# Improbable-AI/walk-these-ways

Measured on AMD Instinct MI355X. Metric: env-steps/sec (sim+PPO), higher is better.
Workload: dtype f32

## Files before the change

### include/go1ppo.h

```cpp
#ifndef GO1PPO_H
#define GO1PPO_H
#include <stdint.h>

#ifdef __cplusplus
extern "C" {
#endif

#define GO1PPO_ABI_VERSION 3
#define GO1PPO_MAX_ACTIONS 32

int go1ppo_elu_fwd(void* y, int64_t rows, int cols, int ld, const void* lat, int lat_ld, int npv, const void* wz,
                   int wz_ld, int lat_cols, void* stream);

int go1ppo_elu_bwd(const void* d, int ld_d, const void* h, int ld_h, int64_t rows, int cols, float* bias_grad, void* out,
                   int ld_out, void* stream);

typedef struct {
  const void* mean;
  const void* value;
  const float* std;
  int32_t head_ld, num_actions;
  int64_t rows;
  const int64_t* idx;
  const float* actions;
// ... 112 lines not shown
                    int64_t count1, float gscale, const float* partial, float max_norm, const float* step, const float* lr,
                    float beta1, float beta2, float eps, void* body, int64_t n_body, float* tail, int64_t n_tail, int zero_grad,
                    float* zero_slot, const Go1PpoAdamExtras* extras, void* stream);

int go1ppo_sum_partials(const void* partials, int count, int64_t stride, int64_t rows, int cols, float* out, int zero_rows,
                        int zero_c0, int zero_c1, void* stream);


typedef struct Go1PpoGemmArgs {
  const void* A; const void* B; void* C; const float* bias; const void* H;
  int32_t M, N, K, lda, ldb, ldc, ldh, epilogue, elu_c0, elu_c1;
  int32_t elu_skip_c0, elu_skip_c1;
  int32_t bias_bf16, _pad;
} Go1PpoGemmArgs;
int go1ppo_gemm_nt(const Go1PpoGemmArgs* args, void* stream);
int go1ppo_gemm_nt_pair(const Go1PpoGemmArgs* a, const Go1PpoGemmArgs* b, void* stream);

int go1ppo_wgrad_tn_plan(Go1PpoWgradProblem* problems, int count);
int go1ppo_wgrad_tn_batched(const Go1PpoWgradProblem* device_problems, int count, int total_workgroups, void* stream);

#define GO1PPO_MLP2_MAX_NETS 3
typedef struct {
  void* x;
  const void* W2; const void* b2;
  const void* W3; const void* b3;
  void* z2;
  void* out;
  int64_t rows;
  int32_t ld_x, ld_z2, ld_out, elu_input;
} Go1PpoMlp2Fwd;
int go1ppo_mlp2_fwd(const Go1PpoMlp2Fwd* nets, int count, void* stream);

typedef struct {
  const void* d_out;
  const void* z2; const void* h;
  const void* W2; const void* W3;
  void* d_z2;
  void* d_x;
  int64_t rows;
  int32_t ld_dout, ld_z2, ld_h, ld_dz2, ld_dx, _pad;
} Go1PpoMlp2Bwd;
int go1ppo_mlp2_bwd(const Go1PpoMlp2Bwd* nets, int count, void* stream);

typedef struct {
  void* x;
  const void* W2; const void* b2;
  const void* W3; const void* b3;
  void* z2;
  void* out;
  void* d_out;
  void* d_z2;
  void* d_x;
  int64_t rows;
  int32_t ld_x, ld_z2, ld_out, ld_dout, ld_dz2, ld_dx, elu_input, _pad;
} Go1PpoMlp2Tail;

#define GO1PPO_TAIL_MAX_ACTIONS 12
int go1ppo_mlp2_tail_ppo(const Go1PpoMlp2Tail* nets, const Go1PpoLossArgs* loss, void* stream);

typedef struct {
  const float* target;
  const int64_t* idx;
  int64_t num_train;
  int32_t npv, selective;
  float* d_pred_bias;
  float* train_loss;
// ... 11 lines not shown
```

### walk-these-ways_amd/csrc/go1ppo_mlp.h

```cpp
#pragma once

#define MLP2_K1 256
#define MLP2_N2 128
#define MLP2_N3 64
#define MLP2_BM 64
#define MLP2_WAVES 16
#define MLP2_THREADS (64 * MLP2_WAVES)
#define MLP2_IMG (128 * 128)

struct Mlp2FwdArgs { Go1PpoMlp2Fwd net[GO1PPO_MLP2_MAX_NETS]; };
struct Mlp2BwdArgs { Go1PpoMlp2Bwd net[GO1PPO_MLP2_MAX_NETS]; };

__device__ __forceinline__ int swz_row(int row) { return row & 15; }
__device__ __forceinline__ int swz_red(int row) { return 2 * ((row & 3) | (((row >> 3) & 1) << 2)); }

template <bool RED>
__device__ __forceinline__ void dma_weights(const bf16_t* W, int rows, int cols, bf16_t* img, int wave, int lane) {
  const int windows = cols >> 7, count = (rows >> 2) * windows;
  for (int idx = wave; idx < count; idx += MLP2_WAVES) {
    const int win = idx % windows, blk = idx / windows;
    const int row = blk * 4 + (lane >> 4);
    const int chunk = (lane & 15) ^ (RED ? swz_red(row) : swz_row(row));
    glds16(W + (int64_t)row * cols + win * 128 + chunk * 8, img + win * MLP2_IMG + blk * 4 * 128);
  }
}

__device__ __forceinline__ uint2 pack_bf4(const float (&v)[4]) {
  f32x2 lo = {v[0], v[1]}, hi = {v[2], v[3]};
  uint2 o;
  o.x = __builtin_bit_cast(uint32_t, __builtin_convertvector(lo, bf16x2_t));
  o.y = __builtin_bit_cast(uint32_t, __builtin_convertvector(hi, bf16x2_t));
  return o;
}
__device__ __forceinline__ void unpack_bf4(uint2 r, float (&v)[4]) {
  v[0] = __uint_as_float(r.x << 16); v[1] = __uint_as_float(r.x & 0xffff0000u);
  v[2] = __uint_as_float(r.y << 16); v[3] = __uint_as_float(r.y & 0xffff0000u);
}
__device__ __forceinline__ bf16x8_t lds_b128(const bf16_t* img, int byte_off) {
  return *reinterpret_cast<const bf16x8_t*>(reinterpret_cast<const char*>(img) + byte_off);
}
__device__ __forceinline__ bf16x8_t lds_tr_operand(const bf16_t* img, int byte_off) {
  typedef __attribute__((address_space(3))) s16x4_t lds_s16x4_t;
  const char* p = reinterpret_cast<const char*>(img) + byte_off;
  s16x4_t lo = __builtin_amdgcn_ds_read_tr16_b64_v4i16((lds_s16x4_t*)(p));
  s16x4_t hi = __builtin_amdgcn_ds_read_tr16_b64_v4i16((lds_s16x4_t*)(p + 4 * 256));
  s16x8_t v = __builtin_shufflevector(lo, hi, 0, 1, 2, 3, 4, 5, 6, 7);
  return __builtin_bit_cast(bf16x8_t, v);
}

__global__ __launch_bounds__(MLP2_THREADS, 1) void mlp2_fwd_kernel(Mlp2FwdArgs A) {
  __shared__ __attribute__((aligned(1024))) bf16_t W2i[2 * MLP2_IMG];
  __shared__ __attribute__((aligned(1024))) bf16_t W3i[64 * 128];
  __shared__ __attribute__((aligned(1024))) bf16_t Ai[2 * 64 * 128];
  __shared__ __attribute__((aligned(1024))) bf16_t Z2i[64 * 128];
  const Go1PpoMlp2Fwd& N = A.net[blockIdx.y];
  const int tiles = (int)((N.rows + MLP2_BM - 1) / MLP2_BM);
  if ((int)blockIdx.x >= tiles) return;
  const int t = threadIdx.x, wave = t >> 6, lane = t & 63, r = lane & 15, g = lane >> 4;
  dma_weights<false>((const bf16_t*)N.W2, MLP2_N2, MLP2_K1, W2i, wave, lane);
  dma_weights<false>((const bf16_t*)N.W3, MLP2_N3, MLP2_N2, W3i, wave, lane);
  bf16_t* x = (bf16_t*)N.x;
  bf16_t* z2 = (bf16_t*)N.z2;
  bf16_t* out = (bf16_t*)N.out;
  const int tx = g ^ r;
  int foff[4];
#pragma unroll
  for (int a = 0; a < 4; a++) foff[a] = r * 256 + (((4 * a) ^ tx) << 4);
  const int nf2 = wave >> 1, mp = (wave & 1) * 2, nf3 = wave & 3, m3 = wave >> 2;
  float bias2[4], bias3[4];
  unpack_bf4(*reinterpret_cast<const uint2*>((const bf16_t*)N.b2 + nf2 * 16 + 4 * g), bias2);
  unpack_bf4(*reinterpret_cast<const uint2*>((const bf16_t*)N.b3 + nf3 * 16 + 4 * g), bias3);

  Bf8 v[2];
  auto fetch = [&](int tile) {
#pragma unroll
    for (int j = 0; j < 2; j++) {
      const int p = t + MLP2_THREADS * j, row = p >> 5, ch = p & 31;
      int64_t grow = (int64_t)tile * MLP2_BM + row;
      grow = grow < N.rows ? grow : N.rows - 1;
      v[j] = *reinterpret_cast<const Bf8*>(x + grow * N.ld_x + ch * 8);
    }
  };
  fetch(blockIdx.x);
  bool first = true;
  for (int tile = blockIdx.x; tile < tiles; tile += gridDim.x) {
    const int64_t row0 = (int64_t)tile * MLP2_BM;
#pragma unroll
    for (int j = 0; j < 2; j++) {
      const int p = t + MLP2_THREADS * j, row = p >> 5, ch = p & 31;
      if (N.elu_input) {
        float f[8];
#pragma unroll
        for (int e = 0; e < 8; e++) f[e] = elu1(bf2f(v[j].v[e]));
        v[j] = pack_bf8(f);
        if (row0 + row < N.rows) *reinterpret_cast<Bf8*>(x + (row0 + row) * N.ld_x + ch * 8) = v[j];
      }
      *reinterpret_cast<Bf8*>(reinterpret_cast<char*>(Ai + (ch >> 4) * 64 * 128) + row * 256 + (((ch & 15) ^ swz_row(row)) << 4)) = v[j];
    }
    if (first) asm volatile("s_waitcnt vmcnt(0)" ::: "memory");
    first = false;
    __syncthreads();
    if (tile + (int)gridDim.x < tiles) fetch(tile + gridDim.x);
    {
      f32x4 acc[2] = {f32x4{0.f, 0.f, 0.f, 0.f}, f32x4{0.f, 0.f, 0.f, 0.f}};
#pragma unroll
      for (int ks = 0; ks < MLP2_K1 / 32; ks++) {
        const int win = ks >> 2, off = foff[ks & 3];
        const bf16x8_t w = lds_b128(W2i + win * MLP2_IMG + nf2 * 16 * 128, off);
#pragma unroll
        for (int m = 0; m < 2; m++)
          acc[m] = __builtin_amdgcn_mfma_f32_16x16x32_bf16(w, lds_b128(Ai + win * 64 * 128 + (mp + m) * 16 * 128, off), acc[m], 0, 0, 0);
      }
      const int n0 = nf2 * 16 + 4 * g;
#pragma unroll
      for (int m = 0; m < 2; m++) {
        const int row = (mp + m) * 16 + r;
        float o4[4];
#pragma unroll
        for (int e = 0; e < 4; e++) o4[e] = elu1(acc[m][e] + bias2[e]);
        const uint2 o = pack_bf4(o4);
        if (row0 + row < N.rows) *reinterpret_cast<uint2*>(z2 + (row0 + row) * N.ld_z2 + n0) = o;
        *reinterpret_cast<uint2*>(reinterpret_cast<char*>(Z2i) + row * 256 + (((n0 >> 3) ^ swz_row(row)) << 4) + ((n0 >> 2) & 1) * 8) = o;
      }
    }
    __syncthreads();
    {
      f32x4 acc = f32x4{0.f, 0.f, 0.f, 0.f};
#pragma unroll
      for (int ks = 0; ks < MLP2_N2 / 32; ks++)
        acc = __builtin_amdgcn_mfma_f32_16x16x32_bf16(lds_b128(W3i + nf3 * 16 * 128, foff[ks]), lds_b128(Z2i + m3 * 16 * 128, foff[ks]), acc, 0, 0, 0);
      const int n0 = nf3 * 16 + 4 * g, row = m3 * 16 + r;
      float o4[4];
#pragma unroll
      for (int e = 0; e < 4; e++) o4[e] = acc[e] + bias3[e];
      if (row0 + row < N.rows) *reinterpret_cast<uint2*>(out + (row0 + row) * N.ld_out + n0) = pack_bf4(o4);
    }
  }
}

__global__ __launch_bounds__(MLP2_THREADS, 1) void mlp2_bwd_kernel(Mlp2BwdArgs A) {
  __shared__ __attribute__((aligned(1024))) bf16_t W3t[64 * 128];
  __shared__ __attribute__((aligned(1024))) bf16_t W2t[2 * MLP2_IMG];
  __shared__ __attribute__((aligned(1024))) bf16_t D3i[64 * 128];
  __shared__ __attribute__((aligned(1024))) bf16_t D2i[64 * 128];
  __shared__ __attribute__((aligned(1024))) bf16_t Hi[2 * 64 * 128];
  const Go1PpoMlp2Bwd& N = A.net[blockIdx.y];
  const int tiles = (int)((N.rows + MLP2_BM - 1) / MLP2_BM);
  if ((int)blockIdx.x >= tiles) return;
  const int t = threadIdx.x, wave = t >> 6, lane = t & 63, r = lane & 15, g = lane >> 4;
  dma_weights<true>((const bf16_t*)N.W3, MLP2_N3, MLP2_N2, W3t, wave, lane);
  dma_weights<true>((const bf16_t*)N.W2, MLP2_N2, MLP2_K1, W2t, wave, lane);
  const bf16_t* d = (const bf16_t*)N.d_out;
  const bf16_t* z2 = (const bf16_t*)N.z2;
  const bf16_t* hin = (const bf16_t*)N.h;
  bf16_t* dz2 = (bf16_t*)N.d_z2;
  bf16_t* dx = (bf16_t*)N.d_x;
  const int tx = g ^ r;
  int foff[4];
#pragma unroll
  for (int a = 0; a < 4; a++) foff[a] = r * 256 + (((4 * a) ^ tx) << 4);
  const int troff = (g * 8 + (r >> 2)) * 256 + ((r & 3) >> 1) * 16 + (r & 1) * 8;
  const int swb = 32 * ((r >> 2) | ((g & 1) << 2));
  const int kf2 = wave >> 1, mp = (wave & 1) * 2;
  const int w3off = troff + (((kf2 * 16) * 2) ^ swb);
  const bf16_t* w2img = W2t + (wave >> 3) * MLP2_IMG;
  const int w2off = troff + ((((wave & 7) * 16) * 2) ^ swb);
  const int hch = t & 31;
#define MLP2_HROW(j) ((t + (j) * MLP2_THREADS) >> 5)
  const int zrow = t >> 4, zch = t & 15, drow = (t >> 3) & 63, dch = t & 7;
#define MLP2_HSLOT(j) ((hch >> 4) * (64 * 128 * 2) + MLP2_HROW(j) * 256 + (((hch & 15) ^ swz_row(MLP2_HROW(j))) << 4))
// ... 493 lines not shown
    });
  }
}

template <int AMAX>
__global__ __launch_bounds__(MLP2_THREADS, 1) void mlp2_tail_ppo_kernel(Mlp2TailPpoArgs A) {
  mlp2_tail_body<0, AMAX>(A.net[blockIdx.y], A.loss, Go1PpoMseArgs{});
}
__global__ __launch_bounds__(MLP2_THREADS, 1) void mlp2_tail_mse_kernel(Mlp2TailMseArgs A) {
  mlp2_tail_body<1, 4>(A.net, Go1PpoLossArgs{}, A.mse);
}

static inline bool aligned8(const void* p) { return (reinterpret_cast<uintptr_t>(p) & 7) == 0; }

extern "C" int go1ppo_mlp2_fwd(const Go1PpoMlp2Fwd* nets, int count, void* stream) {
  if (!nets || count <= 0 || count > GO1PPO_MLP2_MAX_NETS) return -1;
  Mlp2FwdArgs A;
  int64_t max_rows = 0;
  for (int i = 0; i < count; i++) {
    const Go1PpoMlp2Fwd& N = nets[i];
    if (!N.x || !N.W2 || !N.b2 || !N.W3 || !N.b3 || !N.z2 || !N.out || N.rows <= 0) return -1;
    if ((N.ld_x & 7) || (N.ld_z2 & 3) || (N.ld_out & 3) || N.ld_x < MLP2_K1 || N.ld_z2 < MLP2_N2 || N.ld_out < MLP2_N3 || !aligned16(N.x) ||
        !aligned16(N.W2) || !aligned16(N.W3) || !aligned8(N.b2) || !aligned8(N.b3) || !aligned8(N.z2) || !aligned8(N.out))
      return -2;
    A.net[i] = N;
    if (N.rows > max_rows) max_rows = N.rows;
  }
  int64_t wgs = (max_rows + MLP2_BM - 1) / MLP2_BM;
  if (wgs > 256 / count) wgs = 256 / count;
  mlp2_fwd_kernel<<<dim3((unsigned)wgs, count), dim3(MLP2_THREADS), 0, (hipStream_t)stream>>>(A);
  return hipGetLastError() == hipSuccess ? 0 : -9;
}

extern "C" int go1ppo_mlp2_bwd(const Go1PpoMlp2Bwd* nets, int count, void* stream) {
  if (!nets || count <= 0 || count > GO1PPO_MLP2_MAX_NETS) return -1;
  Mlp2BwdArgs A;
  int64_t max_rows = 0;
  for (int i = 0; i < count; i++) {
    const Go1PpoMlp2Bwd& N = nets[i];
    if (!N.d_out || !N.z2 || !N.h || !N.W2 || !N.W3 || !N.d_z2 || !N.d_x || N.rows <= 0) return -1;
    if ((N.ld_dout & 7) || (N.ld_z2 & 7) || (N.ld_h & 7) || (N.ld_dz2 & 7) || (N.ld_dx & 7) || N.ld_dout < MLP2_N3 || N.ld_z2 < MLP2_N2 ||
        N.ld_h < MLP2_K1 || N.ld_dz2 < MLP2_N2 || N.ld_dx < MLP2_K1 || !aligned16(N.d_out) || !aligned16(N.W2) || !aligned16(N.W3) ||
        !aligned16(N.z2) || !aligned16(N.h) || !aligned16(N.d_z2) || !aligned16(N.d_x))
      return -2;
    A.net[i] = N;
    if (N.rows > max_rows) max_rows = N.rows;
  }
  int64_t wgs = (max_rows + MLP2_BM - 1) / MLP2_BM;
  if (wgs > 256 / count) wgs = 256 / count;
  mlp2_bwd_kernel<<<dim3((unsigned)wgs, count), dim3(MLP2_THREADS), 0, (hipStream_t)stream>>>(A);
  return hipGetLastError() == hipSuccess ? 0 : -9;
}

static int mlp2_tail_check(const Go1PpoMlp2Tail& N) {
  if (!N.x || !N.W2 || !N.b2 || !N.W3 || !N.b3 || !N.z2 || !N.out || !N.d_out || !N.d_z2 || !N.d_x || N.rows <= 0) return -1;
  if ((N.rows + MLP2_BM - 1) / MLP2_BM > DET_TAIL_MAX_TILES) return -1;
  return 0;
}
static int mlp2_tail_check_shape(const Go1PpoMlp2Tail& N) {
  if ((N.ld_x & 7) || (N.ld_z2 & 7) || (N.ld_dz2 & 7) || (N.ld_dx & 7) || N.ld_x < MLP2_K1 || N.ld_z2 < MLP2_N2 || N.ld_dz2 < MLP2_N2 ||
      N.ld_dx < MLP2_K1 || N.ld_out != MLP2_N3 || N.ld_dout != MLP2_N3 || !aligned16(N.x) || !aligned16(N.W2) || !aligned16(N.W3) ||
      !aligned8(N.b2) || !aligned8(N.b3) || !aligned16(N.z2) || !aligned16(N.out) || !aligned16(N.d_out) || !aligned16(N.d_z2) ||
      !aligned16(N.d_x) || N.d_z2 == N.z2 || N.d_x == N.x)
    return -2;
  return 0;
}
// ... 43 lines not shown
```

### walk-these-ways_amd/go1_gym_learn/ppo_cse/fused.py

```python
import ctypes
import os

import torch

HEAD = 64
_HERE = os.path.dirname(os.path.abspath(__file__))
_LIB_PATH = os.path.normpath(os.path.join(_HERE, "..", "..", "csrc", "libgo1ppo.so"))
_lib = None


class Go1PpoLibraryMissing(RuntimeError):
    pass


class LossArgs(ctypes.Structure):
    _fields_ = [("mean", ctypes.c_void_p), ("value", ctypes.c_void_p), ("std", ctypes.c_void_p),
                ("head_ld", ctypes.c_int32), ("num_actions", ctypes.c_int32), ("rows", ctypes.c_int64),
                ("idx", ctypes.c_void_p), ("actions", ctypes.c_void_p), ("old_mu", ctypes.c_void_p),
                ("old_sigma", ctypes.c_void_p), ("old_logp", ctypes.c_void_p), ("advantages", ctypes.c_void_p),
                ("returns", ctypes.c_void_p), ("old_values", ctypes.c_void_p),
                ("clip_param", ctypes.c_float), ("value_loss_coef", ctypes.c_float), ("entropy_coef", ctypes.c_float),
                ("use_clipped_value_loss", ctypes.c_int32),
                ("d_mean", ctypes.c_void_p), ("d_value", ctypes.c_void_p), ("d_std", ctypes.c_void_p),
                ("d_mean_bias", ctypes.c_void_p), ("d_value_bias", ctypes.c_void_p), ("kl", ctypes.c_void_p),
# ... 5 lines not shown
                ("rows", ctypes.c_int64), ("ld_dz", ctypes.c_int32), ("ld_h", ctypes.c_int32), ("n", ctypes.c_int32),
                ("k", ctypes.c_int32), ("ldw", ctypes.c_int32), ("chunk_rows", ctypes.c_int32), ("wg_offset", ctypes.c_int32),
                ("zero_n", ctypes.c_int32), ("zero_k0", ctypes.c_int32), ("zero_k1", ctypes.c_int32),
                ("partials", ctypes.c_void_p), ("partial_stride", ctypes.c_int64)]


class GradPiece(ctypes.Structure):
    _fields_ = [("begin", ctypes.c_int64), ("count", ctypes.c_int64), ("src", ctypes.c_void_p), ("stride", ctypes.c_int64),
                ("kind", ctypes.c_int32), ("slabs", ctypes.c_int32), ("cols", ctypes.c_int32), ("zero_rows", ctypes.c_int32),
                ("zero_c0", ctypes.c_int32), ("zero_c1", ctypes.c_int32)]


class TailLayer(ctypes.Structure):
    _fields_ = [("W", ctypes.c_void_p), ("bias", ctypes.c_void_p), ("out", ctypes.c_void_p), ("n_out", ctypes.c_int32),
                ("k_in", ctypes.c_int32), ("ld_out", ctypes.c_int32), ("elu", ctypes.c_int32)]


class TailNet(ctypes.Structure):
    _fields_ = [("in_", ctypes.c_void_p), ("rows", ctypes.c_int64), ("ld_in", ctypes.c_int32), ("num_layers", ctypes.c_int32),
                ("elu_in", ctypes.c_int32), ("npv", ctypes.c_int32), ("latent", ctypes.c_void_p), ("wz", ctypes.c_void_p),
                ("lat_ld", ctypes.c_int32), ("wz_ld", ctypes.c_int32),
                ("layer", TailLayer * 4)]


class TailArgs(ctypes.Structure):
    _fields_ = [("num_nets", ctypes.c_int32), ("_pad", ctypes.c_int32), ("net", TailNet * 3)]


class Mlp2Fwd(ctypes.Structure):
    _fields_ = [(n, ctypes.c_void_p) for n in ("x", "W2", "b2", "W3", "b3", "z2", "out")] + [("rows", ctypes.c_int64)] + \
               [(n, ctypes.c_int32) for n in ("ld_x", "ld_z2", "ld_out", "elu_input")]


class Mlp2Bwd(ctypes.Structure):
    _fields_ = [(n, ctypes.c_void_p) for n in ("d_out", "z2", "h", "W2", "W3", "d_z2", "d_x")] + [("rows", ctypes.c_int64)] + \
               [(n, ctypes.c_int32) for n in ("ld_dout", "ld_z2", "ld_h", "ld_dz2", "ld_dx", "_pad")]


class Mlp2Tail(ctypes.Structure):
    _fields_ = [(n, ctypes.c_void_p) for n in ("x", "W2", "b2", "W3", "b3", "z2", "out", "d_out", "d_z2", "d_x")] + [("rows", ctypes.c_int64)] + \
               [(n, ctypes.c_int32) for n in ("ld_x", "ld_z2", "ld_out", "ld_dout", "ld_dz2", "ld_dx", "elu_input", "_pad")]


class MseArgs(ctypes.Structure):
    _fields_ = [("target", ctypes.c_void_p), ("idx", ctypes.c_void_p), ("num_train", ctypes.c_int64), ("npv", ctypes.c_int32),
                ("selective", ctypes.c_int32), ("d_pred_bias", ctypes.c_void_p), ("train_loss", ctypes.c_void_p), ("test_loss", ctypes.c_void_p)]


MLP2_DIMS = (256, 128, 64)
TAIL_MAX_ACTIONS = 12


class GemmArgs(ctypes.Structure):
    _fields_ = [("A", ctypes.c_void_p), ("B", ctypes.c_void_p), ("C", ctypes.c_void_p), ("bias", ctypes.c_void_p),
                ("H", ctypes.c_void_p)] + [(n, ctypes.c_int32) for n in
                                           ("M", "N", "K", "lda", "ldb", "ldc", "ldh", "epilogue", "elu_c0", "elu_c1", "elu_skip_c0", "elu_skip_c1", "bias_bf16", "_pad")]


class _AdamTranspose(ctypes.Structure):
    _fields_ = [("start", ctypes.c_int64), ("rows", ctypes.c_int32), ("cols", ctypes.c_int32), ("dst", ctypes.c_void_p)]


class AdamExtras(ctypes.Structure):
    _fields_ = [("num_transposes", ctypes.c_int32), ("_pad", ctypes.c_int32), ("transpose", _AdamTranspose * 2)]


EXPORTED_SYMBOLS = ["go1ppo_mlp2_fwd", "go1ppo_mlp2_bwd", "go1ppo_mlp2_tail_ppo", "go1ppo_mlp2_tail_mse", "go1ppo_gemm_nt", "go1ppo_gemm_nt_pair", "go1ppo_sum_partials", "go1ppo_wgrad_tn_plan", "go1ppo_wgrad_tn_batched", "go1ppo_tail_fwd", "go1ppo_elu_fwd", "go1ppo_elu_bwd", "go1ppo_loss", "go1ppo_mse", "go1ppo_wgrad", "go1ppo_wgrad_plan",
                    "go1ppo_wgrad_batched", "go1ppo_act",
                    "go1ppo_store_step", "go1ppo_ring_snapshot", "go1ppo_ring_step", "go1ppo_ring_gather", "go1ppo_gae", "go1ppo_normalize", "go1ppo_opt_partials", "go1ppo_opt_prestep",
                    "go1ppo_opt_prestep_pieces", "go1ppo_grad_reduce", "go1ppo_opt_adam", "go1ppo_version"]


def load_library(path=None):
    global _lib
    if _lib is not None and path is None:
        return _lib
    p = path or _LIB_PATH
    if not os.path.exists(p):
        raise Go1PpoLibraryMissing(f"{p} not found: run `python -c 'import __graft_entry__ as g; g.build()'` "
                                   "(hipcc --offload-arch=gfx950); the fused PPO update has no CPU fallback")
    L = ctypes.CDLL(p)
    vp, i32, i64 = ctypes.c_void_p, ctypes.c_int, ctypes.c_int64
    L.go1ppo_elu_fwd.argtypes = [vp, i64, i32, i32, vp, i32, i32, vp, i32, i32, vp]
    L.go1ppo_elu_bwd.argtypes = [vp, i32, vp, i32, i64, i32, vp, vp, i32, vp]
    L.go1ppo_loss.argtypes = [ctypes.POINTER(LossArgs), vp]
    L.go1ppo_mse.argtypes = [vp, i32, vp, i32, vp, i64, i64, i32, vp, vp, vp, vp, vp]
    L.go1ppo_wgrad.argtypes = [vp, i32, vp, i32, i64, i32, i32, vp, i32, vp, vp]
    L.go1ppo_wgrad_plan.argtypes = [ctypes.POINTER(WgradProblem), i32]
    L.go1ppo_tail_fwd.argtypes = [ctypes.POINTER(TailArgs), vp]
    L.go1ppo_gemm_nt.argtypes = [ctypes.POINTER(GemmArgs), vp]
    L.go1ppo_gemm_nt_pair.argtypes = [ctypes.POINTER(GemmArgs), ctypes.POINTER(GemmArgs), vp]
    L.go1ppo_sum_partials.argtypes = [vp, i32, i64, i64, i32, vp, i32, i32, i32, vp]
    L.go1ppo_mlp2_fwd.argtypes = [ctypes.POINTER(Mlp2Fwd), i32, vp]
    L.go1ppo_mlp2_bwd.argtypes = [ctypes.POINTER(Mlp2Bwd), i32, vp]
    L.go1ppo_mlp2_tail_ppo.argtypes = [ctypes.POINTER(Mlp2Tail), ctypes.POINTER(LossArgs), vp]
    L.go1ppo_mlp2_tail_mse.argtypes = [ctypes.POINTER(Mlp2Tail), ctypes.POINTER(MseArgs), vp]
    L.go1ppo_wgrad_batched.argtypes = [vp, i32, i32, vp]
    L.go1ppo_wgrad_tn_plan.argtypes = [ctypes.POINTER(WgradProblem), i32]
    L.go1ppo_wgrad_tn_batched.argtypes = [vp, i32, i32, vp]
    f32 = ctypes.c_float
    L.go1ppo_act.argtypes = [vp, vp, i32, vp, i32, i64, vp, vp, vp, vp, vp, vp, vp]
    L.go1ppo_store_step.argtypes = [vp, vp, vp, vp, vp, f32, i64, vp, vp, vp, vp]
    L.go1ppo_ring_snapshot.argtypes = [vp, i64, i64, i32, i32, vp, vp]
    L.go1ppo_ring_step.argtypes = [vp, vp, vp, vp, i64, i32, i32, i32, i32, vp, vp, vp, vp]
    L.go1ppo_ring_gather.argtypes = [vp, vp, vp, i64, i64, i32, i32, i32, i32, vp, vp]
    L.go1ppo_gae.argtypes = [vp, vp, vp, vp, i32, i64, f32, f32, vp, vp, vp, vp]
    L.go1ppo_normalize.argtypes = [vp, i64, vp, vp]
    L.go1ppo_opt_partials.argtypes = []
    L.go1ppo_opt_prestep.argtypes = [vp, i64, f32, vp, vp, vp, vp, f32, f32, f32, f32, vp]
    L.go1ppo_opt_prestep_pieces.argtypes = [vp, i64, vp, i32, f32, vp, vp, vp, vp, f32, f32, f32, f32, vp]
    L.go1ppo_grad_reduce.argtypes = [vp, vp, i32, vp]
    L.go1ppo_opt_adam.argtypes = [vp, vp, vp, vp, i64, i64, i64, i64, f32, vp, f32, vp, vp, f32, f32, f32, vp, i64, vp, i64, i32, vp,
                                  ctypes.POINTER(AdamExtras), vp]
    for name in EXPORTED_SYMBOLS[:-1]:
        getattr(L, name).restype = ctypes.c_int
    L.go1ppo_version.restype = ctypes.c_char_p
    if path is None:
        _lib = L
    return L


def _stream():
    return torch.cuda.current_stream().cuda_stream


def _chk(rc, what):
# ... 11 lines not shown


def gemm_args(a, b, c, bias=None, elu=None, elu_bwd_of=None, elu_skip=None):
    g = GemmArgs()
    g.A, g.B, g.C, g.bias, g.H = a.data_ptr(), b.data_ptr(), c.data_ptr(), _ptr(bias), _ptr(elu_bwd_of)
    g.M, g.N, g.K, g.lda, g.ldb, g.ldc = a.shape[0], b.shape[0], a.shape[1], _ld(a), _ld(b), _ld(c)
    assert b.shape[1] == g.K and tuple(c.shape) == (g.M, g.N) and (elu is None or elu_bwd_of is None)
    assert a.dtype == b.dtype == c.dtype == torch.bfloat16 and (bias is None or bias.dtype in (torch.float32, torch.bfloat16))
    g.bias_bf16 = int(bias is not None and bias.dtype == torch.bfloat16)
    if elu_bwd_of is not None:
        assert elu_bwd_of.shape == c.shape and elu_bwd_of.dtype == torch.bfloat16
        g.epilogue, g.ldh = 2, _ld(elu_bwd_of)
    elif elu is not None:
        g.epilogue = 1
        g.elu_c0, g.elu_c1 = (0, g.N) if elu is True else elu
        if elu_skip is not None:
            g.elu_skip_c0, g.elu_skip_c1 = elu_skip
    return g


def gemm_nt(lib, a, b, c, bias=None, elu=None, elu_bwd_of=None):
    g = gemm_args(a, b, c, bias, elu, elu_bwd_of)
    _chk(lib.go1ppo_gemm_nt(ctypes.byref(g), _stream()), "go1ppo_gemm_nt")
    return c


def gemm_nt_pair(lib, first, second):
    ga, gb = gemm_args(**first), gemm_args(**second)
    _chk(lib.go1ppo_gemm_nt_pair(ctypes.byref(ga), ctypes.byref(gb), _stream()), "go1ppo_gemm_nt_pair")


class FusedNet:

    def __init__(self, policy, body, grad, M, lib, with_grad, two_streams=True, fused_tails=None):
        assert body.dtype == torch.bfloat16 and body.is_cuda
        self.pol, self.M, self.lib = policy, M, lib
        dev = body.device
        self.P = {name: policy._block(body, name) for name, _ in policy.blocks}
        self.G = {name: policy._block(grad, name) for name, _ in policy.blocks} if grad is not None else None
        self.nd, self.na, self.nc = policy.first
        self.n1 = self.nd + self.na + self.nc
        self.depth = {n: len(l) for n, l in policy.nets.items()}
        bf = dict(device=dev, dtype=torch.bfloat16)
        self.Y1 = torch.zeros(M, self.n1, **bf)
        self.Y1d = torch.zeros(M, self.nd, **bf)
        self.Z = {n: {li: torch.zeros(M, self.P[f"{n}.{li}.W"].shape[0], **bf) for li in range(1, d)}
                  for n, d in self.depth.items()}
        assert policy.npv <= HEAD and self.P["Wz"].shape == (self.na, HEAD)
        self._recording, self._batched, self._plans = None, False, {}
        self._grad = grad
        self.defer_grad_sum = False
        self._rec_pieces, self._slab_ws, self._last_pieces = None, {}, {}
        self._wgrad_tn = M % 64 == 0
        self._tails = self._tails_ad = None
        if fused_tails is None:
            fused_tails = M <= int(os.environ.get("GO1_FUSED_TAILS_MAX_ROWS", "2048"))
        self._elu_on_load = not with_grad
        if fused_tails and self._fused_tails_ok():
            nd, na = self.nd, self.na
            eol = self._elu_on_load
            self._tails = (self._tail_args([("adaptation", self.Y1[:, :nd])], with_grad, elu_in=eol),
                           self._tail_args([("actor", self.Y1[:, nd:nd + na]), ("critic", self.Y1[:, nd + na:])], with_grad, elu_in=eol,
                                           latent_for="actor" if eol else None))
            self._tails_ad = self._tail_args([("adaptation", self.Y1d)], with_grad)
        self._mlp2 = (self._tails is None and os.environ.get("GO1_MLP2", "1") == "1" and self.nd == MLP2_DIMS[0] and
                      all(self.depth[n] >= 3 and tuple(self.P[f"{n}.{self.depth[n] - 2}.W"].shape) == (MLP2_DIMS[1], MLP2_DIMS[0])
                          and tuple(self.P[f"{n}.{self.depth[n] - 1}.W"].shape) == (MLP2_DIMS[2], MLP2_DIMS[1]) for n in self.depth)
                      and self.depth["adaptation"] == 3 and self.depth["actor"] == 4 and self.depth["critic"] == 4)
        self._mlp2_cache = {}
        self._tail_in_loss = False
        na1, nc1 = int(self.P["actor.1.W"].shape[0]), int(self.P["critic.1.W"].shape[0])
        nt_ok = all(v % 64 == 0 for v in (na1, nc1, self.na, self.n1 - self.nd - self.na)) and \
            all(self.P[k].data_ptr() % 16 == 0 for k in ("actor.1.b", "critic.1.b", "actor.1.W", "critic.1.W"))
        pair_ok = nt_ok and na1 == nc1 and self.na == self.n1 - self.nd - self.na
        self._l1_nt = nt_ok
        self._pair = pair_ok
        self._side = torch.cuda.Stream(device=dev) if two_streams else None
        if with_grad:
            self.X = torch.zeros(M, policy.Kp, **bf)
            self.dH1 = {"adaptation": torch.zeros(M, self.nd, **bf), "actor": torch.zeros(M, self.na, **bf),
                        "critic": torch.zeros(M, self.nc, **bf)}
            self.dY1 = torch.zeros(M, self.n1, **bf)
            self.dZ = {n: {li: torch.zeros_like(z) for li, z in zs.items()} for n, zs in self.Z.items()}
            w1_split = next((b for b in (M // 6144, 4, 2) if b >= 2 and M % b == 0 and (M // b) % 64 == 0), 1)
            self._w1_tmp = torch.zeros(w1_split, self.n1, policy.Kp, **bf)
            self._dgrad_nt = self._mlp2 and nt_ok
            self._WT = {n: torch.zeros(self.P[f"{n}.1.W"].shape[1], self.P[f"{n}.1.W"].shape[0], **bf) for n in ("actor", "critic")} \
                if self._dgrad_nt else None
            self._wt_by_optimizer = False
            self.priv_mask = (self.nd + self.na, policy.K + 1, policy.K + 1 + policy.npv)

    def _elu(self, y, lat=None, lat_cols=0):
        wz = self.P["Wz"] if lat is not None else None
        _chk(self.lib.go1ppo_elu_fwd(y.data_ptr(), y.shape[0], y.shape[1], _ld(y), _ptr(lat), _ld(lat) if lat is not None else 0,
                                     self.pol.npv if lat is not None else 0, _ptr(wz), HEAD, lat_cols, _stream()), "go1ppo_elu_fwd")

    def _elu_bwd(self, d, h, bias_grad, out=None):
        out = d if out is None else out
        _chk(self.lib.go1ppo_elu_bwd(d.data_ptr(), _ld(d), _ptr(h), _ld(h) if h is not None else 0, d.shape[0], d.shape[1],
                                     _ptr(bias_grad), out.data_ptr(), _ld(out), _stream()), "go1ppo_elu_bwd")

    def _wgrad(self, dz, h, gW, gb=None, zero=None):
# ... 39 lines not shown
        for li in range(1, d):
            z = self.Z[net][li]
            torch.addmm(P[f"{net}.{li}.b"], h, P[f"{net}.{li}.W"].t(), out=z)
            if li < d - 1:
                self._elu(z)
            h = z
        return h

    def forward(self, x):
        nd, na = self.nd, self.na
        if self._mlp2:
            return self._forward_mlp2(x)
        torch.mm(x, self.P["W1"].t(), out=self.Y1)
        if self._tails is not None:
            ta, tac = self._tails
            if not self._elu_on_load:
                self._elu(self.Y1[:, :nd])
            _chk(self.lib.go1ppo_tail_fwd(ctypes.byref(ta), _stream()), "go1ppo_tail_fwd")
            latent = self.Z["adaptation"][self.depth["adaptation"] - 1]
            if not self._elu_on_load:
                self._elu(self.Y1[:, nd:], latent, na)
            _chk(self.lib.go1ppo_tail_fwd(ctypes.byref(tac), _stream()), "go1ppo_tail_fwd")
            return self.Z["actor"][self.depth["actor"] - 1], self.Z["critic"][self.depth["critic"] - 1], latent
        self._elu(self.Y1[:, :nd])
        latent = self._tail("adaptation", self.Y1[:, :nd])
        self._elu(self.Y1[:, nd:], latent, na)
        with self._branch():
            value = self._tail("critic", self.Y1[:, nd + na:])
        mean = self._tail("actor", self.Y1[:, nd:nd + na])
        self._join()
        return mean, value, latent

    def _mlp2_fwd(self, key, items, elu_input=1):
        key = ("fwd", key, elu_input)
        if key not in self._mlp2_cache:
            arr = (Mlp2Fwd * len(items))()
            for a, (net, x) in zip(arr, items):
                d = self.depth[net]
                W2, W3, z2, out = self.P[f"{net}.{d - 2}.W"], self.P[f"{net}.{d - 1}.W"], self.Z[net][d - 2], self.Z[net][d - 1]
                a.x, a.W2, a.b2, a.W3, a.b3 = x.data_ptr(), W2.data_ptr(), self.P[f"{net}.{d - 2}.b"].data_ptr(), W3.data_ptr(), self.P[f"{net}.{d - 1}.b"].data_ptr()
                a.z2, a.out, a.rows, a.ld_x, a.ld_z2, a.ld_out, a.elu_input = z2.data_ptr(), out.data_ptr(), x.shape[0], _ld(x), _ld(z2), _ld(out), int(elu_input)
            self._mlp2_cache[key] = (arr, len(items))
        arr, n = self._mlp2_cache[key]
        _chk(self.lib.go1ppo_mlp2_fwd(arr, n, _stream()), "go1ppo_mlp2_fwd")

    def _mlp2_bwd(self, key, items):
        key = ("bwd", key)
        if key not in self._mlp2_cache:
            arr = (Mlp2Bwd * len(items))()
            for a, (net, h, d_x) in zip(arr, items):
                d = self.depth[net]
                d_out, z2, d_z2 = self.dZ[net][d - 1], self.Z[net][d - 2], self.dZ[net][d - 2]
                a.d_out, a.z2, a.h, a.W2, a.W3 = d_out.data_ptr(), z2.data_ptr(), h.data_ptr(), self.P[f"{net}.{d - 2}.W"].data_ptr(), self.P[f"{net}.{d - 1}.W"].data_ptr()
                a.d_z2, a.d_x, a.rows = d_z2.data_ptr(), d_x.data_ptr(), h.shape[0]
                a.ld_dout, a.ld_z2, a.ld_h, a.ld_dz2, a.ld_dx = _ld(d_out), _ld(z2), _ld(h), _ld(d_z2), _ld(d_x)
            self._mlp2_cache[key] = (arr, len(items))
        arr, n = self._mlp2_cache[key]
        _chk(self.lib.go1ppo_mlp2_bwd(arr, n, _stream()), "go1ppo_mlp2_bwd")

    def _mlp2_tail(self, key, items):
        key = ("tail", key)
        if key not in self._mlp2_cache:
            arr = (Mlp2Tail * len(items))()
            for a, (net, x, d_x) in zip(arr, items):
                d = self.depth[net]
                W2, W3, z2, out = self.P[f"{net}.{d - 2}.W"], self.P[f"{net}.{d - 1}.W"], self.Z[net][d - 2], self.Z[net][d - 1]
                d_out, d_z2 = self.dZ[net][d - 1], self.dZ[net][d - 2]
                a.x, a.W2, a.b2, a.W3, a.b3 = x.data_ptr(), W2.data_ptr(), self.P[f"{net}.{d - 2}.b"].data_ptr(), W3.data_ptr(), self.P[f"{net}.{d - 1}.b"].data_ptr()
                a.z2, a.out, a.d_out, a.d_z2, a.d_x, a.rows = z2.data_ptr(), out.data_ptr(), d_out.data_ptr(), d_z2.data_ptr(), d_x.data_ptr(), x.shape[0]
                a.ld_x, a.ld_z2, a.ld_out, a.ld_dout, a.ld_dz2, a.ld_dx, a.elu_input = _ld(x), _ld(z2), _ld(out), _ld(d_out), _ld(d_z2), _ld(d_x), 1
            self._mlp2_cache[key] = arr
        return self._mlp2_cache[key]

    def _tail_ok(self, arr):
        for a in arr:
            if a.ld_out != HEAD or a.ld_dout != HEAD or a.ld_x % 8 or a.ld_z2 % 8 or a.ld_dz2 % 8 or a.ld_dx % 8 or a.d_x == a.x or a.d_z2 == a.z2:
                return False
            if any(p % 16 for p in (a.x, a.W2, a.W3, a.z2, a.out, a.d_out, a.d_z2, a.d_x)) or a.b2 % 8 or a.b3 % 8:
                return False
        return True

    def tail_ppo_fused(self, num_actions):
        if not (self._mlp2 and self.G is not None and 0 < num_actions <= TAIL_MAX_ACTIONS):
            return False
        Z, dZ = self.Z, self.dZ
        return self._tail_ok(self._mlp2_tail("ac", [("actor", Z["actor"][1], dZ["actor"][1]), ("critic", Z["critic"][1], dZ["critic"][1])]))

    def tail_adaptation_fused(self):
        if not (self._mlp2 and self.G is not None):
            return False
        return self._tail_ok(self._mlp2_tail("adaptation_only", [("adaptation", self.Y1d, self.dH1["adaptation"])]))

    def _forward_mlp2(self, x):
        P, Z, nd, na = self.P, self.Z, self.nd, self.na
        torch.mm(x, P["W1"].t(), out=self.Y1)
        self._mlp2_fwd("adaptation", [("adaptation", self.Y1[:, :nd])])
        latent = Z["adaptation"][2]
        self._elu(self.Y1[:, nd:], latent, na)
        if self._l1_nt and self._pair:
            gemm_nt_pair(self.lib, dict(a=self.Y1[:, nd:nd + na], b=P["actor.1.W"], c=Z["actor"][1], bias=P["actor.1.b"]),
                         dict(a=self.Y1[:, nd + na:], b=P["critic.1.W"], c=Z["critic"][1], bias=P["critic.1.b"]))
        elif self._l1_nt:
            with self._branch():
                gemm_nt(self.lib, self.Y1[:, nd + na:], P["critic.1.W"], Z["critic"][1], P["critic.1.b"])
            gemm_nt(self.lib, self.Y1[:, nd:nd + na], P["actor.1.W"], Z["actor"][1], P["actor.1.b"])
        else:
            with self._branch():
                torch.addmm(P["critic.1.b"], self.Y1[:, nd + na:], P["critic.1.W"].t(), out=Z["critic"][1])
            torch.addmm(P["actor.1.b"], self.Y1[:, nd:nd + na], P["actor.1.W"].t(), out=Z["actor"][1])
        self._join()
        if not self._tail_in_loss:
            self._mlp2_fwd("ac", [("actor", Z["actor"][1]), ("critic", Z["critic"][1])])
        return Z["actor"][3], Z["critic"][3], latent

    def _backward_mlp2(self, x):
        nd, na = self.nd, self.na
        P, G, Z, dZ, Y1, dY1, dH1 = self.P, self.G, self.Z, self.dZ, self.Y1, self.dY1, self.dH1
        cols = {"adaptation": slice(0, nd), "actor": slice(nd, nd + na), "critic": slice(nd + na, self.n1)}
        if not self._tail_in_loss:
            self._mlp2_bwd("ac", [("actor", Z["actor"][1], dZ["actor"][1]), ("critic", Z["critic"][1], dZ["critic"][1])])
        for net in ("actor", "critic"):
            self._wgrad(dZ[net][3], Z[net][2], G[f"{net}.3.W"], None)
            self._wgrad(dZ[net][2], Z[net][1], G[f"{net}.2.W"], G[f"{net}.2.b"])
            self._wgrad(dZ[net][1], Y1[:, cols[net]], G[f"{net}.1.W"], G[f"{net}.1.b"])
        if self._dgrad_nt and self._pair and self._wt_by_optimizer:
            gemm_nt_pair(self.lib, dict(a=dZ["actor"][1], b=self._WT["actor"], c=dY1[:, cols["actor"]], elu_bwd_of=Y1[:, cols["actor"]]),
                         dict(a=dZ["critic"][1], b=self._WT["critic"], c=dY1[:, cols["critic"]], elu_bwd_of=Y1[:, cols["critic"]]))
        elif self._dgrad_nt:
            with self._branch():
                if not self._wt_by_optimizer:
                    self._WT["critic"].copy_(P["critic.1.W"].t())
# ... 353 lines not shown
```

Measured before the change: 5.332 million.

## Fold latent-injection ELU pass into adaptation MLP2 forward kernel

Adds a templated variant of the adaptation MLP2 forward kernel that, besides computing the adaptation latent, also applies the latent-weight injection and ELU to the rest of the first-layer activation block. Each workgroup finishes its own tile's latent-dependent columns from LDS and streams the latent-free columns of another tile while it waits on memory. This removes a separate ELU kernel launch and a round trip of the latent through global memory. It is enabled by default only for large batches, and falls back to the old path if alignment checks fail. The cost is more LDS use, software prefetch of the next tile is moved later, and the kernel code is considerably more complex.

```diff
diff --git a/include/go1ppo.h b/include/go1ppo.h
--- a/include/go1ppo.h
+++ b/include/go1ppo.h
@@ -168,6 +168,13 @@
 int go1ppo_mlp2_fwd(const Go1PpoMlp2Fwd* nets, int count, void* stream);
 
 typedef struct {
+  void* y;
+  const void* wz;
+  int32_t cols, ld, lat_cols, npv, wz_ld, _pad;
+} Go1PpoEluBlock;
+int go1ppo_mlp2_fwd_elu(const Go1PpoMlp2Fwd* net, const Go1PpoEluBlock* blk, void* stream);
+
+typedef struct {
   const void* d_out;
   const void* z2; const void* h;
   const void* W2; const void* W3;
diff --git a/walk-these-ways_amd/csrc/go1ppo_mlp.h b/walk-these-ways_amd/csrc/go1ppo_mlp.h
--- a/walk-these-ways_amd/csrc/go1ppo_mlp.h
+++ b/walk-these-ways_amd/csrc/go1ppo_mlp.h
@@ -48,12 +48,20 @@
   return __builtin_bit_cast(bf16x8_t, v);
 }
 
-__global__ __launch_bounds__(MLP2_THREADS, 1) void mlp2_fwd_kernel(Mlp2FwdArgs A) {
+#define ELU_U 4
+#define ELU_WZ_LDS_COLS 2048
+struct Mlp2FwdEluArgs { Go1PpoMlp2Fwd net; Go1PpoEluBlock blk; };
+struct EluWalk { int row, ch; };
+struct EluCols { int c0, cpr, q, rm; };
+
+template <bool FOLD>
+__device__ __forceinline__ void mlp2_fwd_body(const Go1PpoMlp2Fwd& N, const Go1PpoEluBlock& E) {
   __shared__ __attribute__((aligned(1024))) bf16_t W2i[2 * MLP2_IMG];
   __shared__ __attribute__((aligned(1024))) bf16_t W3i[64 * 128];
   __shared__ __attribute__((aligned(1024))) bf16_t Ai[2 * 64 * 128];
   __shared__ __attribute__((aligned(1024))) bf16_t Z2i[64 * 128];
-  const Go1PpoMlp2Fwd& N = A.net[blockIdx.y];
+  __shared__ __attribute__((aligned(16))) bf16_t Hd[FOLD ? 64 * 64 : 8];
+  __shared__ __attribute__((aligned(16))) uint32_t Wl[FOLD ? ELU_WZ_LDS_COLS : 4];
   const int tiles = (int)((N.rows + MLP2_BM - 1) / MLP2_BM);
   if ((int)blockIdx.x >= tiles) return;
   const int t = threadIdx.x, wave = t >> 6, lane = t & 63, r = lane & 15, g = lane >> 4;
@@ -71,6 +79,92 @@
   unpack_bf4(*reinterpret_cast<const uint2*>((const bf16_t*)N.b2 + nf2 * 16 + 4 * g), bias2);
   unpack_bf4(*reinterpret_cast<const uint2*>((const bf16_t*)N.b3 + nf3 * 16 + 4 * g), bias3);
 
+  bf16_t* y = (bf16_t*)E.y;
+  const bf16_t* wz = (const bf16_t*)E.wz;
+  const int lc = FOLD ? (wz && E.lat_cols > 0 ? (E.lat_cols < E.cols ? E.lat_cols : E.cols) : 0) : 0;
+  auto ecols = [&](int c0, int c1) {
+    EluCols G;
+    G.c0 = c0; G.cpr = (c1 - c0) >> 3;
+    G.q = G.cpr ? MLP2_THREADS / G.cpr : 0; G.rm = MLP2_THREADS - G.q * G.cpr;
+    return G;
+  };
+  const EluCols GL = ecols(0, lc), GF = ecols(lc, FOLD ? E.cols : 0);
+  const bool wz_lds = FOLD && E.npv == 2 && lc <= ELU_WZ_LDS_COLS;
+  auto walk0 = [&](const EluCols& G) { EluWalk k; k.row = G.cpr ? t / G.cpr : MLP2_BM; k.ch = G.cpr ? t - k.row * G.cpr : 0; return k; };
+  auto walk = [&](EluWalk& k, const EluCols& G) {
+    k.row += G.q; k.ch += G.rm;
+    if (k.ch >= G.cpr) { k.ch -= G.cpr; k.row++; }
+  };
+  const EluWalk kL0 = walk0(GL), kF0 = walk0(GF);
+  auto restart = [&](EluWalk k) { asm volatile("" : "+v"(k.row), "+v"(k.ch)); return k; };
+  auto eload = [&](const EluCols& G, int64_t row0, EluWalk k, auto& w) {
+    constexpr int U = (int)(sizeof(w) / sizeof(Bf8));
+#pragma unroll
+    for (int u = 0; u < U; u++) {
+      if (k.row < MLP2_BM && row0 + k.row < N.rows) w[u] = *reinterpret_cast<const Bf8*>(y + (row0 + k.row) * E.ld + G.c0 + k.ch * 8);
+      walk(k, G);
+    }
+  };
+  auto efinish = [&](const EluCols& G, int64_t row0, EluWalk& k, const auto& w, int lat) {
+#pragma clang fp contract(off)
+    constexpr int U = (int)(sizeof(w) / sizeof(Bf8));
+#pragma unroll
+    for (int u = 0; u < U; u++) {
+      if (k.row < MLP2_BM && row0 + k.row < N.rows) {
+        float f[8];
+#pragma unroll
+        for (int e = 0; e < 8; e++) f[e] = bf2f(w[u].v[e]);
+        if (lat) {
+          const int c = k.ch * 8;
+          if (lat == 1) {
+            const uint4 lo = *reinterpret_cast<const uint4*>(Wl + c), hi = *reinterpret_cast<const uint4*>(Wl + c + 4);
+            const uint32_t wp[8] = {lo.x, lo.y, lo.z, lo.w, hi.x, hi.y, hi.z, hi.w};
+            const uint32_t p = *reinterpret_cast<const uint32_t*>(Hd + k.row * 64);
+            const float l0 = __uint_as_float(p << 16), l1 = __uint_as_float(p & 0xffff0000u);
+#pragma unroll
+            for (int e = 0; e < 8; e++) f[e] = fmaf(l1, __uint_as_float(wp[e] & 0xffff0000u), fmaf(l0, __uint_as_float(wp[e] << 16), f[e]));
+          } else {
+#pragma unroll
+            for (int e = 0; e < 8; e++) {
+              const bf16_t* wc = wz + (int64_t)(c + e) * E.wz_ld;
+#pragma unroll 1
+              for (int q = 0; q < E.npv; q++) f[e] = fmaf(bf2f(Hd[k.row * 64 + q]), bf2f(wc[q]), f[e]);
+            }
+          }
+        }
+#pragma unroll
+        for (int e = 0; e < 8; e++) f[e] = elu1(f[e]);
+        put16_wt(y + (row0 + k.row) * E.ld + G.c0 + k.ch * 8, pack_bf8(f));
+      }
+      walk(k, G);
+      __builtin_amdgcn_sched_barrier(0);
+    }
+  };
+  auto erest = [&](const EluCols& G, int64_t row0, EluWalk& k) {
+    while (k.row < MLP2_BM) {
+      Bf8 w[1];
+      eload(G, row0, k, w);
+      efinish(G, row0, k, w, 2);
+    }
+  };
+  auto estream = [&](int64_t row0, EluWalk& k, Bf8 (&a)[ELU_U / 2], Bf8 (&b)[ELU_U / 2]) {
+    auto ahead = [&](EluWalk n) {
+#pragma unroll
+      for (int u = 0; u < ELU_U / 2; u++) walk(n, GF);
+      return n;
+    };
+    while (k.row < MLP2_BM) {
+      eload(GF, row0, ahead(k), b);
+      efinish(GF, row0, k, a, 0);
+      if (k.row >= MLP2_BM) break;
+      eload(GF, row0, ahead(k), a);
+      efinish(GF, row0, k, b, 0);
+    }
+  };
+  if (wz_lds)
+    for (int c = t; c < lc; c += MLP2_THREADS) Wl[c] = *reinterpret_cast<const uint32_t*>(wz + (int64_t)c * E.wz_ld);
+  int funit = (int)(gridDim.x - 1 - blockIdx.x);
+
   Bf8 v[2];
   auto fetch = [&](int tile) {
 #pragma unroll
@@ -100,7 +194,14 @@
     if (first) asm volatile("s_waitcnt vmcnt(0)" ::: "memory");
     first = false;
     __syncthreads();
-    if (tile + (int)gridDim.x < tiles) fetch(tile + gridDim.x);
+    if (!FOLD && tile + (int)gridDim.x < tiles) fetch(tile + gridDim.x);
+    Bf8 wL[ELU_U], wFa[ELU_U / 2], wFb[ELU_U / 2];
+    EluWalk kL = kL0, kF = kF0;
+    if (FOLD) {
+      kL = restart(kL0);
+      kF = restart(kF0);
+      if (wz_lds) eload(GL, row0, kL, wL);
+    }
     {
       f32x4 acc[2] = {f32x4{0.f, 0.f, 0.f, 0.f}, f32x4{0.f, 0.f, 0.f, 0.f}};
 #pragma unroll
@@ -133,9 +234,39 @@
       float o4[4];
 #pragma unroll
       for (int e = 0; e < 4; e++) o4[e] = acc[e] + bias3[e];
-      if (row0 + row < N.rows) *reinterpret_cast<uint2*>(out + (row0 + row) * N.ld_out + n0) = pack_bf4(o4);
-    }
-  }
+      const uint2 o = pack_bf4(o4);
+      if (row0 + row < N.rows) *reinterpret_cast<uint2*>(out + (row0 + row) * N.ld_out + n0) = o;
+      if (FOLD) *reinterpret_cast<uint2*>(Hd + row * 64 + n0) = o;
+    }
+    if (FOLD) {
+      const bool free_unit = funit < tiles;
+      const int64_t frow0 = (int64_t)funit * MLP2_BM;
+      if (free_unit) eload(GF, frow0, kF, wFa);
+      __syncthreads();
+      if (wz_lds) efinish(GL, row0, kL, wL, 1);
+      erest(GL, row0, kL);
+      if (tile + (int)gridDim.x < tiles) fetch(tile + gridDim.x);
+      if (free_unit) {
+        estream(frow0, kF, wFa, wFb);
+        funit += gridDim.x;
+      }
+    }
+  }
+  if (FOLD) {
+    for (; funit < tiles; funit += gridDim.x) {
+      EluWalk kF = restart(kF0);
+      Bf8 wFa[ELU_U / 2], wFb[ELU_U / 2];
+      eload(GF, (int64_t)funit * MLP2_BM, kF, wFa);
+      estream((int64_t)funit * MLP2_BM, kF, wFa, wFb);
+    }
+  }
+}
+
+__global__ __launch_bounds__(MLP2_THREADS, 1) void mlp2_fwd_kernel(Mlp2FwdArgs A) {
+  mlp2_fwd_body<false>(A.net[blockIdx.y], Go1PpoEluBlock{});
+}
+__global__ __launch_bounds__(MLP2_THREADS, 1) void mlp2_fwd_elu_kernel(Mlp2FwdEluArgs A) {
+  mlp2_fwd_body<true>(A.net, A.blk);
 }
 
 __global__ __launch_bounds__(MLP2_THREADS, 1) void mlp2_bwd_kernel(Mlp2BwdArgs A) {
@@ -695,6 +826,28 @@
   return hipGetLastError() == hipSuccess ? 0 : -9;
 }
 
+extern "C" int go1ppo_mlp2_fwd_elu(const Go1PpoMlp2Fwd* net, const Go1PpoEluBlock* blk, void* stream) {
+  if (!net || !blk) return -1;
+  const Go1PpoMlp2Fwd& N = *net;
+  const Go1PpoEluBlock& E = *blk;
+  if (!N.x || !N.W2 || !N.b2 || !N.W3 || !N.b3 || !N.z2 || !N.out || N.rows <= 0 || N.rows > INT32_MAX || !E.y || E.cols <= 0) return -1;
+  if ((N.ld_x & 7) || (N.ld_z2 & 3) || (N.ld_out & 3) || N.ld_x < MLP2_K1 || N.ld_z2 < MLP2_N2 || N.ld_out < MLP2_N3 || !aligned16(N.x) ||
+      !aligned16(N.W2) || !aligned16(N.W3) || !aligned8(N.b2) || !aligned8(N.b3) || !aligned8(N.z2) || !aligned8(N.out))
+    return -2;
+  if ((E.cols & 7) || (E.ld & 7) || E.ld < E.cols || (E.lat_cols & 7) || E.lat_cols < 0 || !aligned16(E.y)) return -2;
+  if (E.lat_cols > 0) {
+    if (!E.wz || E.npv <= 0 || E.npv > MLP2_N3) return -2;
+    if (E.npv == 2 && (((N.ld_out | E.wz_ld) & 1) || (reinterpret_cast<uintptr_t>(E.wz) & 3))) return -2;
+  }
+  Mlp2FwdEluArgs A;
+  A.net = N;
+  A.blk = E;
+  int64_t wgs = (N.rows + MLP2_BM - 1) / MLP2_BM;
+  if (wgs > 256) wgs = 256;
+  mlp2_fwd_elu_kernel<<<dim3((unsigned)wgs), dim3(MLP2_THREADS), 0, (hipStream_t)stream>>>(A);
+  return hipGetLastError() == hipSuccess ? 0 : -9;
+}
+
 extern "C" int go1ppo_mlp2_bwd(const Go1PpoMlp2Bwd* nets, int count, void* stream) {
   if (!nets || count <= 0 || count > GO1PPO_MLP2_MAX_NETS) return -1;
   Mlp2BwdArgs A;
diff --git a/walk-these-ways_amd/go1_gym_learn/ppo_cse/fused.py b/walk-these-ways_amd/go1_gym_learn/ppo_cse/fused.py
--- a/walk-these-ways_amd/go1_gym_learn/ppo_cse/fused.py
+++ b/walk-these-ways_amd/go1_gym_learn/ppo_cse/fused.py
@@ -61,6 +61,11 @@
                [(n, ctypes.c_int32) for n in ("ld_x", "ld_z2", "ld_out", "elu_input")]
 
 
+class EluBlock(ctypes.Structure):
+    _fields_ = [("y", ctypes.c_void_p), ("wz", ctypes.c_void_p)] + \
+               [(n, ctypes.c_int32) for n in ("cols", "ld", "lat_cols", "npv", "wz_ld", "_pad")]
+
+
 class Mlp2Bwd(ctypes.Structure):
     _fields_ = [(n, ctypes.c_void_p) for n in ("d_out", "z2", "h", "W2", "W3", "d_z2", "d_x")] + [("rows", ctypes.c_int64)] + \
                [(n, ctypes.c_int32) for n in ("ld_dout", "ld_z2", "ld_h", "ld_dz2", "ld_dx", "_pad")]
@@ -77,6 +82,7 @@
 
 
 MLP2_DIMS = (256, 128, 64)
+ELU_FOLD_MIN_ROWS = 256 * 64
 TAIL_MAX_ACTIONS = 12
 
 
@@ -94,7 +100,7 @@
     _fields_ = [("num_transposes", ctypes.c_int32), ("_pad", ctypes.c_int32), ("transpose", _AdamTranspose * 2)]
 
 
-EXPORTED_SYMBOLS = ["go1ppo_mlp2_fwd", "go1ppo_mlp2_bwd", "go1ppo_mlp2_tail_ppo", "go1ppo_mlp2_tail_mse", "go1ppo_gemm_nt", "go1ppo_gemm_nt_pair", "go1ppo_sum_partials", "go1ppo_wgrad_tn_plan", "go1ppo_wgrad_tn_batched", "go1ppo_tail_fwd", "go1ppo_elu_fwd", "go1ppo_elu_bwd", "go1ppo_loss", "go1ppo_mse", "go1ppo_wgrad", "go1ppo_wgrad_plan",
+EXPORTED_SYMBOLS = ["go1ppo_mlp2_fwd", "go1ppo_mlp2_fwd_elu", "go1ppo_mlp2_bwd", "go1ppo_mlp2_tail_ppo", "go1ppo_mlp2_tail_mse", "go1ppo_gemm_nt", "go1ppo_gemm_nt_pair", "go1ppo_sum_partials", "go1ppo_wgrad_tn_plan", "go1ppo_wgrad_tn_batched", "go1ppo_tail_fwd", "go1ppo_elu_fwd", "go1ppo_elu_bwd", "go1ppo_loss", "go1ppo_mse", "go1ppo_wgrad", "go1ppo_wgrad_plan",
                     "go1ppo_wgrad_batched", "go1ppo_act",
                     "go1ppo_store_step", "go1ppo_ring_snapshot", "go1ppo_ring_step", "go1ppo_ring_gather", "go1ppo_gae", "go1ppo_normalize", "go1ppo_opt_partials", "go1ppo_opt_prestep",
                     "go1ppo_opt_prestep_pieces", "go1ppo_grad_reduce", "go1ppo_opt_adam", "go1ppo_version"]
@@ -121,6 +127,7 @@
     L.go1ppo_gemm_nt_pair.argtypes = [ctypes.POINTER(GemmArgs), ctypes.POINTER(GemmArgs), vp]
     L.go1ppo_sum_partials.argtypes = [vp, i32, i64, i64, i32, vp, i32, i32, i32, vp]
     L.go1ppo_mlp2_fwd.argtypes = [ctypes.POINTER(Mlp2Fwd), i32, vp]
+    L.go1ppo_mlp2_fwd_elu.argtypes = [ctypes.POINTER(Mlp2Fwd), ctypes.POINTER(EluBlock), vp]
     L.go1ppo_mlp2_bwd.argtypes = [ctypes.POINTER(Mlp2Bwd), i32, vp]
     L.go1ppo_mlp2_tail_ppo.argtypes = [ctypes.POINTER(Mlp2Tail), ctypes.POINTER(LossArgs), vp]
     L.go1ppo_mlp2_tail_mse.argtypes = [ctypes.POINTER(Mlp2Tail), ctypes.POINTER(MseArgs), vp]
@@ -198,7 +205,7 @@
 
 class FusedNet:
 
-    def __init__(self, policy, body, grad, M, lib, with_grad, two_streams=True, fused_tails=None):
+    def __init__(self, policy, body, grad, M, lib, with_grad, two_streams=True, fused_tails=None, elu_fold=None):
         assert body.dtype == torch.bfloat16 and body.is_cuda
         self.pol, self.M, self.lib = policy, M, lib
         dev = body.device
@@ -234,6 +241,7 @@
                           and tuple(self.P[f"{n}.{self.depth[n] - 1}.W"].shape) == (MLP2_DIMS[2], MLP2_DIMS[1]) for n in self.depth)
                       and self.depth["adaptation"] == 3 and self.depth["actor"] == 4 and self.depth["critic"] == 4)
         self._mlp2_cache = {}
+        self._elu_fold = self._mlp2 and (M > ELU_FOLD_MIN_ROWS if elu_fold is None else bool(elu_fold))
         self._tail_in_loss = False
         na1, nc1 = int(self.P["actor.1.W"].shape[0]), int(self.P["critic.1.W"].shape[0])
         nt_ok = all(v % 64 == 0 for v in (na1, nc1, self.na, self.n1 - self.nd - self.na)) and \
@@ -339,6 +347,10 @@
         return mean, value, latent
 
     def _mlp2_fwd(self, key, items, elu_input=1):
+        arr, n = self._mlp2_fwd_args(key, items, elu_input)
+        _chk(self.lib.go1ppo_mlp2_fwd(arr, n, _stream()), "go1ppo_mlp2_fwd")
+
+    def _mlp2_fwd_args(self, key, items, elu_input):
         key = ("fwd", key, elu_input)
         if key not in self._mlp2_cache:
             arr = (Mlp2Fwd * len(items))()
@@ -348,8 +360,7 @@
                 a.x, a.W2, a.b2, a.W3, a.b3 = x.data_ptr(), W2.data_ptr(), self.P[f"{net}.{d - 2}.b"].data_ptr(), W3.data_ptr(), self.P[f"{net}.{d - 1}.b"].data_ptr()
                 a.z2, a.out, a.rows, a.ld_x, a.ld_z2, a.ld_out, a.elu_input = z2.data_ptr(), out.data_ptr(), x.shape[0], _ld(x), _ld(z2), _ld(out), int(elu_input)
             self._mlp2_cache[key] = (arr, len(items))
-        arr, n = self._mlp2_cache[key]
-        _chk(self.lib.go1ppo_mlp2_fwd(arr, n, _stream()), "go1ppo_mlp2_fwd")
+        return self._mlp2_cache[key]
 
     def _mlp2_bwd(self, key, items):
         key = ("bwd", key)
@@ -398,12 +409,28 @@
             return False
         return self._tail_ok(self._mlp2_tail("adaptation_only", [("adaptation", self.Y1d, self.dH1["adaptation"])]))
 
+    def _mlp2_fwd_elu(self):
+        key = ("fwd_elu",)
+        if key not in self._mlp2_cache:
+            arr, _ = self._mlp2_fwd_args("adaptation", [("adaptation", self.Y1[:, :self.nd])], 1)
+            y, blk = self.Y1[:, self.nd:], EluBlock()
+            blk.y, blk.wz, blk.cols, blk.ld, blk.lat_cols, blk.npv, blk.wz_ld = y.data_ptr(), self.P["Wz"].data_ptr(), y.shape[1], _ld(y), self.na, self.pol.npv, HEAD
+            self._mlp2_cache[key] = (arr, blk)
+        arr, blk = self._mlp2_cache[key]
+        rc = self.lib.go1ppo_mlp2_fwd_elu(arr, ctypes.byref(blk), _stream())
+        if rc == -2:
+            self._elu_fold = False
+            return False
+        _chk(rc, "go1ppo_mlp2_fwd_elu")
+        return True
+
     def _forward_mlp2(self, x):
         P, Z, nd, na = self.P, self.Z, self.nd, self.na
         torch.mm(x, P["W1"].t(), out=self.Y1)
-        self._mlp2_fwd("adaptation", [("adaptation", self.Y1[:, :nd])])
         latent = Z["adaptation"][2]
-        self._elu(self.Y1[:, nd:], latent, na)
+        if not (self._elu_fold and self._mlp2_fwd_elu()):
+            self._mlp2_fwd("adaptation", [("adaptation", self.Y1[:, :nd])])
+            self._elu(self.Y1[:, nd:], latent, na)
         if self._l1_nt and self._pair:
             gemm_nt_pair(self.lib, dict(a=self.Y1[:, nd:nd + na], b=P["actor.1.W"], c=Z["actor"][1], bias=P["actor.1.b"]),
                          dict(a=self.Y1[:, nd + na:], b=P["critic.1.W"], c=Z["critic"][1], bias=P["critic.1.b"]))
```

Result: no change. 5.325 million (-0.1%).
